# vitasoftAI/ImageRetrievalResearch

Measured on AMD Instinct MI355X. Metric: images/sec embed + queries/sec top-k@100k-gallery, EffNet-B3a 224^2, higher is better.
Workload: dtype bf16

## Files before the change

### imageretrievalresearch_amd/csrc/conv_kernels.hip

```cpp
#include "ops.h"

#include <stdlib.h>
#include <type_traits>

namespace mi355 {

typedef float f32x4 __attribute__((ext_vector_type(4)));
typedef unsigned u32x4 __attribute__((ext_vector_type(4)));
typedef unsigned u32x2 __attribute__((ext_vector_type(2)));

__device__ __forceinline__ void unpack8(u32x4 v, float* f) {
    f[0] = __uint_as_float(v.x << 16); f[1] = __uint_as_float(v.x & 0xffff0000u);
    f[2] = __uint_as_float(v.y << 16); f[3] = __uint_as_float(v.y & 0xffff0000u);
    f[4] = __uint_as_float(v.z << 16); f[5] = __uint_as_float(v.z & 0xffff0000u);
    f[6] = __uint_as_float(v.w << 16); f[7] = __uint_as_float(v.w & 0xffff0000u);
}
__device__ __forceinline__ u32x4 pack8(const float* f) {
    u32x4 o;
    o.x = pack2bf(f[0], f[1]); o.y = pack2bf(f[2], f[3]); o.z = pack2bf(f[4], f[5]); o.w = pack2bf(f[6], f[7]);
    return o;
}

__global__ __launch_bounds__(256) void k_stem(const float* __restrict__ x, const float* __restrict__ w,
                                              const float* __restrict__ bias, bf16_t* __restrict__ out, int H, int W,
                                              int Ho, int Wo, int Cout, int act) {
    const int b = blockIdx.z;
    const int ox = blockIdx.x * 32 + (threadIdx.x & 31);
    const int oy = blockIdx.y * 8 + (threadIdx.x >> 5);
    if (ox >= Wo || oy >= Ho) return;
    float p[27];
    const float* xb = x + (size_t)b * 3 * H * W;
#pragma unroll
    for (int ky = 0; ky < 3; ++ky) {
        const int iy = oy * 2 - 1 + ky;
#pragma unroll
        for (int kx = 0; kx < 3; ++kx) {
            const int ix = ox * 2 - 1 + kx;
            const bool ok = (iy >= 0 && iy < H && ix >= 0 && ix < W);
#pragma unroll
            for (int ci = 0; ci < 3; ++ci)
                p[(ky * 3 + kx) * 3 + ci] = ok ? xb[((size_t)ci * H + iy) * W + ix] : 0.f;
        }
    }
    bf16_t* o = out + (((size_t)b * Ho + oy) * Wo + ox) * Cout;
    for (int c0 = 0; c0 < Cout; c0 += 8) {
        float acc[8];
#pragma unroll
        for (int j = 0; j < 8; ++j) acc[j] = bias[c0 + j];
#pragma unroll
        for (int t = 0; t < 27; ++t) {
            const f32x4 w0 = *reinterpret_cast<const f32x4*>(&w[t * Cout + c0]);
            const f32x4 w1 = *reinterpret_cast<const f32x4*>(&w[t * Cout + c0 + 4]);
            acc[0] += p[t] * w0.x; acc[1] += p[t] * w0.y; acc[2] += p[t] * w0.z; acc[3] += p[t] * w0.w;
            acc[4] += p[t] * w1.x; acc[5] += p[t] * w1.y; acc[6] += p[t] * w1.z; acc[7] += p[t] * w1.w;
        }
        MI355_ACT_DISPATCH(act, {
_Pragma("unroll")
            for (int j = 0; j < 8; ++j) acc[j] = act_c<ACT>(acc[j]);
        })
        *reinterpret_cast<u32x4*>(o + c0) = pack8(acc);
    }
}

int launch_stem(const float* x, const float* w, const float* bias, bf16_t* out, int B, int H, int W, int Cout, int act,
                hipStream_t st) {
    MI355_REQUIRE(Cout % 8 == 0 && Cout <= 256, "stem: Cout=%d must be a multiple of 8 and <= 256", Cout);
    const int Ho = (H + 2 - 3) / 2 + 1, Wo = (W + 2 - 3) / 2 + 1;
    dim3 grid(cdiv(Wo, 32), cdiv(Ho, 8), B);
    hipLaunchKernelGGL(k_stem, grid, dim3(256), 0, st, x, w, bias, out, H, W, Ho, Wo, Cout, act);
    MI355_LAUNCH_CHECK();
    return OK;
}

struct StemU8Args {
    const unsigned char* img;
    int h, w, S, hp, vp, fill;
    float mean[3], stdv[3];
    const float* cw;
};
struct StemU8RaggedArgs : StemU8Args {
    const int64_t* desc;
    int b0;
};

template <bool CONV_INPUT, bool RAGGED>
__global__ __launch_bounds__(256) void k_stem_u8(const std::conditional_t<RAGGED, StemU8RaggedArgs, StemU8Args> a,
                                                 const float* __restrict__ w,
                                                 const float* __restrict__ bias, bf16_t* __restrict__ out, int Ho, int Wo,
                                                 int Cout, int act) {
    constexpr int PW = 67, PH = 19, CWD = 65, CHT = 17;
    __shared__ float scw[81];
    __shared__ float Pt[CONV_INPUT ? PH * PW * 3 : 1];
    __shared__ float Ct[CONV_INPUT ? CHT * CWD * 3 : 1];
    const int b = blockIdx.z;
    const int lx = threadIdx.x & 31, ly = threadIdx.x >> 5;
    const int ox = blockIdx.x * 32 + lx;
    const int oy = blockIdx.y * 8 + ly;
    StemU8Args g = a;
    if constexpr (RAGGED) {
        const int64_t* d = a.desc + (size_t)(a.b0 + b) * 3;
        g.img = a.img + d[0]; g.h = (int)d[1]; g.w = (int)d[2];
        g.hp = (a.S - g.w) / 2; g.vp = (a.S - g.h) / 2;
    }
    const unsigned char* ib = RAGGED ? g.img : g.img + (size_t)b * g.h * g.w * 3;
    auto pre = [&](int y, int x, int c) -> float {
        if (y < 0 || y >= g.S || x < 0 || x >= g.S) return 0.f;
        const int iy = y - g.vp, ix = x - g.hp;
        int v = g.fill;
        if (iy >= 0 && iy < g.h && ix >= 0 && ix < g.w) v = ib[((size_t)iy * g.w + ix) * 3 + c];
        return __fdiv_rn(__fsub_rn(__fdiv_rn((float)v, 255.0f), g.mean[c]), g.stdv[c]);
    };
    float p[27];
    if (!CONV_INPUT) {
        if (ox >= Wo || oy >= Ho) return;
#pragma unroll
        for (int ky = 0; ky < 3; ++ky)
#pragma unroll
            for (int kx = 0; kx < 3; ++kx)
#pragma unroll
                for (int ci = 0; ci < 3; ++ci) p[(ky * 3 + kx) * 3 + ci] = pre(oy * 2 - 1 + ky, ox * 2 - 1 + kx, ci);
    } else {
        if (threadIdx.x < 81) scw[threadIdx.x] = g.cw[threadIdx.x];
        const int y0 = blockIdx.y * 16 - 2, x0 = blockIdx.x * 64 - 2;
        for (int i = threadIdx.x; i < PH * PW; i += 256) {
            const int r = i / PW, c = i - r * PW;
#pragma unroll
            for (int ci = 0; ci < 3; ++ci) Pt[i * 3 + ci] = pre(y0 + r, x0 + c, ci);
        }
        __syncthreads();
        for (int i = threadIdx.x; i < CHT * CWD; i += 256) {
            const int r = i / CWD, c = i - r * CWD;
            const int y = y0 + 1 + r, x = x0 + 1 + c;
            float acc[3] = {0.f, 0.f, 0.f};
#pragma unroll
            for (int ci = 0; ci < 3; ++ci)
#pragma unroll
                for (int ky2 = 0; ky2 < 3; ++ky2)
#pragma unroll
                    for (int kx2 = 0; kx2 < 3; ++kx2) {
                        const float v = Pt[((r + ky2) * PW + c + kx2) * 3 + ci];
#pragma unroll
                        for (int co = 0; co < 3; ++co) acc[co] += v * scw[((co * 3 + ci) * 3 + ky2) * 3 + kx2];
                    }
            const bool in = y >= 0 && y < g.S && x >= 0 && x < g.S;
#pragma unroll
            for (int co = 0; co < 3; ++co) Ct[i * 3 + co] = in ? silu_f(acc[co]) : 0.f;
        }
        __syncthreads();
        if (ox >= Wo || oy >= Ho) return;
#pragma unroll
        for (int ky = 0; ky < 3; ++ky)
#pragma unroll
            for (int kx = 0; kx < 3; ++kx)
#pragma unroll
                for (int co = 0; co < 3; ++co) p[(ky * 3 + kx) * 3 + co] = Ct[((ly * 2 + ky) * CWD + lx * 2 + kx) * 3 + co];
    }
    bf16_t* o = out + (((size_t)b * Ho + oy) * Wo + ox) * Cout;
    for (int c0 = 0; c0 < Cout; c0 += 8) {
        float acc[8];
#pragma unroll
        for (int j = 0; j < 8; ++j) acc[j] = bias[c0 + j];
#pragma unroll
        for (int t = 0; t < 27; ++t) {
            const f32x4 w0 = *reinterpret_cast<const f32x4*>(&w[t * Cout + c0]);
            const f32x4 w1 = *reinterpret_cast<const f32x4*>(&w[t * Cout + c0 + 4]);
            acc[0] += p[t] * w0.x; acc[1] += p[t] * w0.y; acc[2] += p[t] * w0.z; acc[3] += p[t] * w0.w;
            acc[4] += p[t] * w1.x; acc[5] += p[t] * w1.y; acc[6] += p[t] * w1.z; acc[7] += p[t] * w1.w;
        }
        MI355_ACT_DISPATCH(act, {
_Pragma("unroll")
            for (int j = 0; j < 8; ++j) acc[j] = act_c<ACT>(acc[j]);
        })
        *reinterpret_cast<u32x4*>(o + c0) = pack8(acc);
    }
}

int launch_stem_u8(const unsigned char* img, int h, int w, int fill, const float* mean, const float* stdv,
                   const float* conv_w, const float* sw, const float* bias, bf16_t* out, int B, int Cout, int act,
                   hipStream_t st, const int64_t* desc, int b0) {
    MI355_REQUIRE(Cout % 8 == 0 && Cout <= 256, "stem: Cout=%d must be a multiple of 8 and <= 256", Cout);
    StemU8RaggedArgs r{};
    StemU8Args& a = r;
    a.img = img; a.h = h; a.w = w; a.S = h > w ? h : w; a.hp = (a.S - w) / 2; a.vp = (a.S - h) / 2; a.fill = fill;
    for (int c = 0; c < 3; ++c) { a.mean[c] = mean[c]; a.stdv[c] = stdv[c]; }
    a.cw = conv_w;
    r.desc = desc; r.b0 = b0;
    const int Ho = (a.S + 2 - 3) / 2 + 1, Wo = Ho;
    dim3 grid(cdiv(Wo, 32), cdiv(Ho, 8), B);
    if (desc) {
        if (conv_w) hipLaunchKernelGGL((k_stem_u8<true, true>), grid, dim3(256), 0, st, r, sw, bias, out, Ho, Wo, Cout, act);
        else hipLaunchKernelGGL((k_stem_u8<false, true>), grid, dim3(256), 0, st, r, sw, bias, out, Ho, Wo, Cout, act);
    } else if (conv_w) {
        hipLaunchKernelGGL((k_stem_u8<true, false>), grid, dim3(256), 0, st, a, sw, bias, out, Ho, Wo, Cout, act);
    } else {
        hipLaunchKernelGGL((k_stem_u8<false, false>), grid, dim3(256), 0, st, a, sw, bias, out, Ho, Wo, Cout, act);
    }
    MI355_LAUNCH_CHECK();
    return OK;
}

#ifndef MI355_DW_PX
#define MI355_DW_PX 4
#endif
constexpr int DW_PX = MI355_DW_PX;

int dw_pool_blocks(int Ho, int Wo, int C) {
    const long items = (long)(C / 8) * cdiv(Wo, DW_PX) * Ho;
    return cdiv(items, 256);
}

template <int KS, int S>
__global__ __launch_bounds__(256) void k_dwconv(const bf16_t* __restrict__ in, const bf16_t* __restrict__ w,
                                                const float* __restrict__ bias, bf16_t* __restrict__ out,
                                                float* __restrict__ pool_partial, int B, int nblk, int H, int W, int C,
                                                int Ho, int Wo, int act) {
    constexpr int PAD = KS / 2;
    constexpr int IW = (DW_PX - 1) * S + KS;
    __shared__ float red[256][8];
    const int CG = C >> 3;
    const int strips = (Wo + DW_PX - 1) / DW_PX;
    const int xcd = blockIdx.x & 7;
    const int seq = blockIdx.x >> 3;
    const int b = xcd + 8 * (seq / nblk);
    const int blk = seq - (seq / nblk) * nblk;
    if (b >= B) return;
    const long item = (long)blk * 256 + threadIdx.x;
    const long nitems = (long)CG * strips * Ho;
    const bool live = item < nitems;
    const int cg = (int)(item % CG);
    const long rest = item / CG;
    const int sx = (int)(rest % strips);
    const int oy = (int)(rest / strips);
    const int ox0 = sx * DW_PX;
    const int c0 = cg * 8;

    float acc[DW_PX][8];
    float psum[8];
#pragma unroll
    for (int j = 0; j < 8; ++j) psum[j] = 0.f;

    if (live) {
        float bs[8];
        {
            const f32x4 b0 = *reinterpret_cast<const f32x4*>(bias + c0);
            const f32x4 b1 = *reinterpret_cast<const f32x4*>(bias + c0 + 4);
            bs[0] = b0.x; bs[1] = b0.y; bs[2] = b0.z; bs[3] = b0.w; bs[4] = b1.x; bs[5] = b1.y; bs[6] = b1.z; bs[7] = b1.w;
        }
#pragma unroll
        for (int p = 0; p < DW_PX; ++p)
#pragma unroll
            for (int j = 0; j < 8; ++j) acc[p][j] = bs[j];

        const bf16_t* inb = in + (size_t)b * H * W * C + c0;
#pragma unroll
        for (int ky = 0; ky < KS; ++ky) {
            const int iy = oy * S - PAD + ky;
            if (iy < 0 || iy >= H) continue;
            float wk[KS][8];
#pragma unroll
            for (int kx = 0; kx < KS; ++kx)
                unpack8(*reinterpret_cast<const u32x4*>(w + (size_t)(ky * KS + kx) * C + c0), wk[kx]);
            const bf16_t* row = inb + (size_t)iy * W * C;
#pragma unroll
            for (int i = 0; i < IW; ++i) {
                const int ix = ox0 * S - PAD + i;
                if (ix < 0 || ix >= W) continue;
                float v[8];
                unpack8(*reinterpret_cast<const u32x4*>(row + (size_t)ix * C), v);
#pragma unroll
                for (int p = 0; p < DW_PX; ++p) {
                    const int kx = i - p * S;
                    if (kx >= 0 && kx < KS) {
#pragma unroll
                        for (int j = 0; j < 8; ++j) acc[p][j] += wk[kx][j] * v[j];
                    }
                }
            }
        }
        bf16_t* o = out + (((size_t)b * Ho + oy) * Wo + ox0) * C + c0;
        MI355_ACT_DISPATCH(act, {
_Pragma("unroll")
            for (int p = 0; p < DW_PX; ++p)
_Pragma("unroll")
                for (int j = 0; j < 8; ++j) acc[p][j] = act_c<ACT>(acc[p][j]);
        })
#pragma unroll
        for (int p = 0; p < DW_PX; ++p) {
            if (ox0 + p < Wo) {
#pragma unroll
                for (int j = 0; j < 8; ++j) psum[j] += acc[p][j];
                if (C >= 64) __builtin_nontemporal_store(pack8(acc[p]), reinterpret_cast<u32x4*>(o + (size_t)p * C));
                else *reinterpret_cast<u32x4*>(o + (size_t)p * C) = pack8(acc[p]);
            }
        }
    }

    if (pool_partial != nullptr) {
#pragma unroll
        for (int j = 0; j < 8; ++j) red[threadIdx.x][j] = psum[j];
        __syncthreads();
        const int ncg = CG < 256 ? CG : 256;
        if ((int)threadIdx.x < ncg) {
            float s[8];
#pragma unroll
            for (int j = 0; j < 8; ++j) s[j] = 0.f;
            for (int u = threadIdx.x; u < 256; u += CG) {
#pragma unroll
                for (int j = 0; j < 8; ++j) s[j] += red[u][j];
            }
            const int my_cg = (int)(((long)blk * 256 + threadIdx.x) % CG);
            float* pp = pool_partial + ((size_t)b * nblk + blk) * C + my_cg * 8;
            *reinterpret_cast<f32x4*>(pp) = (f32x4){s[0], s[1], s[2], s[3]};
            *reinterpret_cast<f32x4*>(pp + 4) = (f32x4){s[4], s[5], s[6], s[7]};
        }
        if (CG > 256) {
            const int first = (int)(((long)blk * 256) % CG);
            for (int t = 256 + threadIdx.x; t < CG; t += 256) {
                const int z = (first + t) % CG;
                float* pp = pool_partial + ((size_t)b * nblk + blk) * C + z * 8;
                *reinterpret_cast<f32x4*>(pp) = (f32x4){0.f, 0.f, 0.f, 0.f};
                *reinterpret_cast<f32x4*>(pp + 4) = (f32x4){0.f, 0.f, 0.f, 0.f};
            }
        }
    }
}

template <int KS, int PX>
__global__ __launch_bounds__(256) void k_dw_tiled(const bf16_t* __restrict__ in, const bf16_t* __restrict__ w,
                                                  const float* __restrict__ bias, bf16_t* __restrict__ out,
                                                  float* __restrict__ pool_partial, int H, int W, int C, int TH, int CGC,
                                                  int nbands, int act) {
    constexpr int PAD = KS / 2;
    constexpr int IW = PX - 1 + KS;
    extern __shared__ __attribute__((aligned(16))) bf16_t tile[];
    const int b = blockIdx.y;
    const int band = blockIdx.x % nbands, chunk = blockIdx.x / nbands;
    const int oy0 = band * TH;
    const int th = min(TH, H - oy0);
    const int IH = TH + KS - 1, EW = W + 2 * PAD + (PX - 1);
    const int cg0 = chunk * CGC;
    const int CG = C >> 3;
    const int ncg = min(CGC, CG - cg0);
    const int PS = CGC * 8;
    const bf16_t* inb = in + (size_t)b * H * W * C;
    for (int id = threadIdx.x; id < IH * EW * CGC; id += 256) {
        const int cg = id % CGC;
        const int px = id / CGC;
        const int r = px / EW, x = px - r * EW;
        const int iy = oy0 - PAD + r, ix = x - PAD;
        u32x4 v = {0u, 0u, 0u, 0u};
        if (cg < ncg && iy >= 0 && iy < H && ix >= 0 && ix < W)
            v = *reinterpret_cast<const u32x4*>(inb + ((size_t)iy * W + ix) * C + (cg0 + cg) * 8);
        *reinterpret_cast<u32x4*>(&tile[(size_t)px * PS + cg * 8]) = v;
    }
    __syncthreads();

    const int strips = (W + PX - 1) / PX;
    const int nitems = CGC * strips * th;
    float psum[8];
#pragma unroll
    for (int j = 0; j < 8; ++j) psum[j] = 0.f;
    for (int item = threadIdx.x; item < nitems; item += 256) {
        const int cg = item % CGC;
        const int rest = item / CGC;
        const int sx = rest % strips, oyl = rest / strips;
        if (cg >= ncg) continue;
        const int ox0 = sx * PX;
        const int c0 = (cg0 + cg) * 8;
        float acc[PX][8];
        {
            const f32x4 b0 = *reinterpret_cast<const f32x4*>(bias + c0);
            const f32x4 b1 = *reinterpret_cast<const f32x4*>(bias + c0 + 4);
// ... 585 lines not shown
```

### imageretrievalresearch_amd/csrc/gemm_bf16.hip

```cpp
#include "ops.h"
#include "../../include/mi355_retrieval.h"

#include <stdlib.h>

namespace mi355 {

typedef __bf16 bf16x8 __attribute__((ext_vector_type(8)));
typedef float f32x4 __attribute__((ext_vector_type(4)));
typedef unsigned u32x4 __attribute__((ext_vector_type(4)));
typedef unsigned u32x2 __attribute__((ext_vector_type(2)));

__device__ __forceinline__ float lo_bf(unsigned u) { return __uint_as_float(u << 16); }
__device__ __forceinline__ float hi_bf(unsigned u) { return __uint_as_float(u & 0xffff0000u); }

__device__ __forceinline__ u32x4 gate_chunk(u32x4 v, const float* __restrict__ gp, int relu6) {
    const f32x4 g0 = *reinterpret_cast<const f32x4*>(gp);
    const f32x4 g1 = *reinterpret_cast<const f32x4*>(gp + 4);
    float f[8] = {lo_bf(v.x) * g0.x, hi_bf(v.x) * g0.y, lo_bf(v.y) * g0.z, hi_bf(v.y) * g0.w,
                  lo_bf(v.z) * g1.x, hi_bf(v.z) * g1.y, lo_bf(v.w) * g1.z, hi_bf(v.w) * g1.w};
    if (relu6) {
#pragma unroll
        for (int i = 0; i < 8; ++i) f[i] = fminf(fmaxf(f[i], 0.f), 6.f);
    }
    u32x4 o;
// ... 647 lines not shown
        if (row < Npad && c * 8 < g.ldw) v = *reinterpret_cast<const u32x4*>(g.W + (size_t)row * g.ldw + c * 8);
        *reinterpret_cast<u32x4*>(&Wsh[row * WLD + c * 8]) = v;
    }
    for (int n = tid; n < NT * 16; n += 512) sbias[n] = n < Npad ? g.bias[n] : 0.f;
    for (int id = lane; id < 16 * (ALD / 8); id += 64) *reinterpret_cast<u32x4*>(&As[id * 8]) = (u32x4){0u, 0u, 0u, 0u};
    __syncthreads();

    const int fr = lane & 15, fq = lane >> 4;
    const int kc = g.K >> 3;
    const int nchunk = 16 * kc;
    const int ntiles = (g.M + 15) >> 4;
    const int stride = gridDim.x * NW;
    int img = -1;
    u32x4 sv[KST];
    auto stage_load = [&](int tile) {
#pragma unroll
        for (int i = 0; i < KST; ++i) {
            const int id = min(lane + 64 * i, nchunk - 1);
            const int row = id / kc, c = id - row * kc;
            const int m = min(tile * 16 + row, g.M - 1);
            sv[i] = *reinterpret_cast<const u32x4*>(g.A + (size_t)m * g.lda + c * 8);
        }
        __builtin_amdgcn_sched_barrier(0);
    };
    int tile = blockIdx.x * NW + wave;
    if (tile < ntiles) stage_load(tile);
    for (; tile < ntiles; tile += stride) {
        if (g.gate) {
            const int im = (tile * 16) / g.rows_per_img;
            if (im != img) {
                img = im;
                for (int k4 = lane; k4 * 4 < g.K; k4 += 64)
                    *reinterpret_cast<f32x4*>(&Gs[k4 * 4]) = *reinterpret_cast<const f32x4*>(g.gate + (size_t)im * g.gate_ld + k4 * 4);
            }
        }
#pragma unroll
        for (int i = 0; i < KST; ++i) {
            const int id = lane + 64 * i;
            if (id < nchunk) {
                const int row = id / kc, c = id - row * kc;
                u32x4 v = sv[i];
                if (g.gate) v = gate_chunk(v, Gs + c * 8, g.a_relu6);
                else if (g.a_relu6) v = relu6_chunk(v);
                *reinterpret_cast<u32x4*>(&As[row * ALD + c * 8]) = v;
            }
        }
        if (tile + stride < ntiles) stage_load(tile + stride);
        f32x4 acc[NT];
#pragma unroll
        for (int ni = 0; ni < NT; ++ni) acc[ni] = (f32x4){0.f, 0.f, 0.f, 0.f};
#pragma unroll
        for (int ks = 0; ks < KST; ++ks) {
            const bf16x8 af = *reinterpret_cast<const bf16x8*>(&As[fr * ALD + ks * 32 + fq * 8]);
#pragma unroll
            for (int ni = 0; ni < NT; ++ni) {
                const bf16x8 wf = *reinterpret_cast<const bf16x8*>(&Wsh[(ni * 16 + fr) * WLD + ks * 32 + fq * 8]);
                acc[ni] = __builtin_amdgcn_mfma_f32_16x16x32_bf16(wf, af, acc[ni], 0, 0, 0);
            }
        }
        MI355_ACT_DISPATCH(g.act, {
_Pragma("unroll")
            for (int ni = 0; ni < NT; ++ni) {
                const f32x4 bb = *reinterpret_cast<const f32x4*>(&sbias[ni * 16 + fq * 4]);
                acc[ni].x = act_c<ACT>(acc[ni].x + bb.x); acc[ni].y = act_c<ACT>(acc[ni].y + bb.y);
                acc[ni].z = act_c<ACT>(acc[ni].z + bb.z); acc[ni].w = act_c<ACT>(acc[ni].w + bb.w);
            }
        })
        const int m = tile * 16 + fr;
#pragma unroll
        for (int ni = 0; ni < NT; ++ni) {
            const int n = ni * 16 + fq * 4;
            float v[4] = {acc[ni].x, acc[ni].y, acc[ni].z, acc[ni].w};
            if (g.res && m < g.M && n < g.N) {
                if (n + 3 < g.res_n) {
                    const u32x2 rr = *reinterpret_cast<const u32x2*>(g.res + (size_t)m * g.ldr + n);
                    v[0] += lo_bf(rr.x); v[1] += hi_bf(rr.x); v[2] += lo_bf(rr.y); v[3] += hi_bf(rr.y);
                } else {
#pragma unroll
                    for (int r = 0; r < 4; ++r)
                        if (n + r < g.res_n) v[r] += bf2f(g.res[(size_t)m * g.ldr + n + r]);
                }
            }
            u32x2 o;
            o.x = pack2bf(v[0], v[1]);
            o.y = pack2bf(v[2], v[3]);
            *reinterpret_cast<u32x2*>(&Cs[fr * CLD + n]) = o;
        }
        constexpr int CPR = NT * 2;
#pragma unroll
        for (int i = 0; i < (16 * CPR + 63) / 64; ++i) {
            const int id = lane + 64 * i;
            const int row = id / CPR, c = id - row * CPR;
            const int mm = tile * 16 + row;
            if (id < 16 * CPR && mm < g.M && c * 8 < g.N)
                *reinterpret_cast<u32x4*>((bf16_t*)g.out + (size_t)mm * g.ldo + c * 8) =
                    *reinterpret_cast<const u32x4*>(&Cs[row * CLD + c * 8]);
        }
    }
}

template <int NT, int KST>
static int launch_proj_cfg(const GemmArgs& a, hipStream_t st) {
    constexpr int KP = KST * 32;
    const size_t lds = (size_t)NT * 16 * (KP + 8) * 2 + (size_t)NT * 16 * 4 +
                       (size_t)8 * (16 * (KP + 8) * 2 + 16 * (NT * 16 + 8) * 2 + KP * 4);
    static bool attr_done[MI355_MAX_DEVICES] = {false};
    if (first_time_on_this_device(attr_done)) {
        MI355_CHECK_HIP(hipFuncSetAttribute((const void*)k_proj_lds<NT, KST>, hipFuncAttributeMaxDynamicSharedMemorySize,
                                            160 * 1024));
    }
    const int ntiles = cdiv(a.M, 16);
    int blocks = cdiv(ntiles, 8);
    if (blocks > 256 * 6) blocks = 256 * 6;
    hipLaunchKernelGGL((k_proj_lds<NT, KST>), dim3(blocks), dim3(512), lds, st, a);
    MI355_LAUNCH_CHECK();
    return OK;
}

static int try_launch_proj(const GemmArgs& a, hipStream_t st, int* nt_out) {
    if (a.out_f32 || a.M < (1 << 19) || a.N % 8 || a.ldo % 8 || a.N > 64 || a.K > 288 || a.lda != a.K) return -1;
    if (a.gate && (a.rows_per_img % 16 != 0 || a.gate_ld % 4 != 0)) return -1;
    const int kst = (a.K + 31) / 32, nt = (a.N + 15) / 16;
#define PROJ_CASE(NTV, KSTV) if (nt == NTV && kst == KSTV) { *nt_out = NTV; return launch_proj_cfg<NTV, KSTV>(a, st); }
    PROJ_CASE(2, 1); PROJ_CASE(2, 2); PROJ_CASE(2, 5); PROJ_CASE(2, 6); PROJ_CASE(3, 6); PROJ_CASE(3, 9); PROJ_CASE(2, 9);
    PROJ_CASE(4, 8); PROJ_CASE(3, 5);
#undef PROJ_CASE
    return -1;
}

static int try_launch_stream(const GemmArgs& a, hipStream_t st, int* nt_out) {
    if (a.out_f32 || a.M < 4096 || a.N % 8 || a.ldo % 8 || a.gate || a.a_relu6) return -1;
    const int kst = (a.K + 31) / 32;
    const int nt = (a.N + 15) / 16;
    *nt_out = nt;
    if (kst == 1 && nt == 9) return launch_stream_cfg<9, 1>(a, st);
    if (kst == 1 && nt == 12) return launch_stream_cfg<12, 1>(a, st);
    return -1;
}

constexpr int SK_KC = 256, SK_BM = 64, SK_BN = 64, SK_LD = SK_KC + 8;
constexpr size_t SK_MAX_BYTES = (size_t)64 << 20;

int gemm_splitk_chunks(long M, int rows_per_img, int N, int K) {
    if (M > 16384 || rows_per_img > 196 || K < 512 || N < 64 || N % 8 || gemm_splitk_bytes(M, N, K) > SK_MAX_BYTES) return 0;
    return (K + SK_KC - 1) / SK_KC;
}
size_t gemm_splitk_bytes(long M, int N, int K) {
    return (size_t)((K + SK_KC - 1) / SK_KC) * (size_t)M * (size_t)((N + 15) & ~15) * sizeof(float);
}

__global__ __launch_bounds__(256) void k_gemm_splitk(const GemmArgs g, float* __restrict__ ws) {
    extern __shared__ __attribute__((aligned(16))) bf16_t sksm[];
    bf16_t* As = sksm;
    bf16_t* Ws = sksm + SK_BM * SK_LD;
    const int tid = threadIdx.x, lane = tid & 63, wave = tid >> 6;
    const int n0 = blockIdx.x * SK_BN, m0 = blockIdx.y * SK_BM, k0 = blockIdx.z * SK_KC;
    const int Npad = (g.N + 15) & ~15;
    u32x4 ra[8], rw[8];
#pragma unroll
    for (int i = 0; i < 8; ++i) {
        const int id = tid + 256 * i;
        const int row = id >> 5, c = id & 31;
        const int k = k0 + c * 8;
        const int m = min(m0 + row, g.M - 1), kk = min(k, g.K - 8);
        ra[i] = *reinterpret_cast<const u32x4*>(g.A + (size_t)m * g.lda + kk);
        const int n = min(n0 + row, Npad - 1), kw = min(k, g.ldw - 8);
        rw[i] = *reinterpret_cast<const u32x4*>(g.W + (size_t)n * g.ldw + kw);
    }
#pragma unroll
    for (int i = 0; i < 8; ++i) {
        const int id = tid + 256 * i;
        const int row = id >> 5, c = id & 31;
        const int k = k0 + c * 8;
        u32x4 v = ra[i];
        if (m0 + row < g.M && k < g.K) {
            if (g.gate) v = gate_chunk(v, g.gate + (size_t)((m0 + row) / g.rows_per_img) * g.gate_ld + k, g.a_relu6);
            else if (g.a_relu6) v = relu6_chunk(v);
        } else {
            v = (u32x4){0u, 0u, 0u, 0u};
        }
        *reinterpret_cast<u32x4*>(&As[row * SK_LD + c * 8]) = v;
        u32x4 w = rw[i];
        if (n0 + row >= Npad || k >= g.ldw) w = (u32x4){0u, 0u, 0u, 0u};
        *reinterpret_cast<u32x4*>(&Ws[row * SK_LD + c * 8]) = w;
    }
    __syncthreads();
    const int fr = lane & 15, fq = lane >> 4;
    const int wm = wave >> 1, wn = wave & 1;
    f32x4 acc[2][2];
#pragma unroll
    for (int j = 0; j < 2; ++j)
#pragma unroll
        for (int i = 0; i < 2; ++i) acc[j][i] = (f32x4){0.f, 0.f, 0.f, 0.f};
#pragma unroll
    for (int ks = 0; ks < SK_KC / 32; ++ks) {
        bf16x8 af[2], wf[2];
#pragma unroll
        for (int i = 0; i < 2; ++i) af[i] = *reinterpret_cast<const bf16x8*>(&As[(wm * 32 + i * 16 + fr) * SK_LD + ks * 32 + fq * 8]);
#pragma unroll
        for (int j = 0; j < 2; ++j) wf[j] = *reinterpret_cast<const bf16x8*>(&Ws[(wn * 32 + j * 16 + fr) * SK_LD + ks * 32 + fq * 8]);
#pragma unroll
        for (int j = 0; j < 2; ++j)
#pragma unroll
            for (int i = 0; i < 2; ++i) acc[j][i] = __builtin_amdgcn_mfma_f32_16x16x32_bf16(wf[j], af[i], acc[j][i], 0, 0, 0);
    }
    float* wsk = ws + (size_t)blockIdx.z * g.M * Npad;
#pragma unroll
    for (int i = 0; i < 2; ++i) {
        const int m = m0 + wm * 32 + i * 16 + fr;
#pragma unroll
        for (int j = 0; j < 2; ++j) {
            const int n = n0 + wn * 32 + j * 16 + fq * 4;
            if (m < g.M && n < Npad) *reinterpret_cast<f32x4*>(wsk + (size_t)m * Npad + n) = acc[j][i];
        }
    }
}

__global__ __launch_bounds__(256) void k_splitk_reduce(const GemmArgs g, const float* __restrict__ ws, int nchunks) {
    const int Npad = (g.N + 15) & ~15, n4s = Npad >> 2;
    const long t = (long)blockIdx.x * 256 + threadIdx.x;
    if (t >= (long)g.M * n4s) return;
    const int m = (int)(t / n4s), n = (int)(t - (long)m * n4s) * 4;
    if (n >= g.N) return;
    f32x4 s = *reinterpret_cast<const f32x4*>(ws + (size_t)m * Npad + n);
    for (int c = 1; c < nchunks; ++c) {
        const f32x4 p = *reinterpret_cast<const f32x4*>(ws + ((size_t)c * g.M + m) * Npad + n);
        s.x += p.x; s.y += p.y; s.z += p.z; s.w += p.w;
    }
    const f32x4 bb = *reinterpret_cast<const f32x4*>(g.bias + n);
    float v[4] = {apply_act(s.x + bb.x, g.act), apply_act(s.y + bb.y, g.act), apply_act(s.z + bb.z, g.act), apply_act(s.w + bb.w, g.act)};
    if (g.res) {
#pragma unroll
        for (int r = 0; r < 4; ++r)
            if (n + r < g.res_n) v[r] += bf2f(g.res[(size_t)m * g.ldr + n + r]);
    }
    u32x2 o;
    o.x = pack2bf(v[0], v[1]);
    o.y = pack2bf(v[2], v[3]);
    *reinterpret_cast<u32x2*>((bf16_t*)g.out + (size_t)m * g.ldo + n) = o;
}

static int launch_splitk(const GemmArgs& a, int nchunks, hipStream_t st) {
    const size_t lds = (size_t)(SK_BM + SK_BN) * SK_LD * 2;
    static bool attr_done[MI355_MAX_DEVICES] = {false};
    if (first_time_on_this_device(attr_done)) {
        MI355_CHECK_HIP(hipFuncSetAttribute((const void*)k_gemm_splitk, hipFuncAttributeMaxDynamicSharedMemorySize, (int)lds));
    }
    const int Npad = (a.N + 15) & ~15;
    hipLaunchKernelGGL(k_gemm_splitk, dim3((unsigned)cdiv(Npad, SK_BN), (unsigned)cdiv(a.M, SK_BM), (unsigned)nchunks), dim3(256), lds, st,
                       a, a.splitk_ws);
    MI355_LAUNCH_CHECK();
    hipLaunchKernelGGL(k_splitk_reduce, dim3((unsigned)cdiv((long)a.M * (Npad / 4), 256)), dim3(256), 0, st, a,
                       (const float*)a.splitk_ws, nchunks);
    MI355_LAUNCH_CHECK();
    return OK;
}

static int pick_nt(int N, int max_nt = 12) {
    static const int opts[] = {2, 3, 4, 6, 8, 9, 12};
    int best = 2;
    double best_cost = 1e30;
    for (int nt : opts) {
        if (nt > max_nt) continue;
        const int bn = nt * 16;
        const int tiles = (N + bn - 1) / bn;
        const double cost = (double)tiles * bn * (1.0 + 24.0 / bn) + 8.0 * tiles;
        if (cost < best_cost) { best_cost = cost; best = nt; }
    }
    return best;
}

template <int WM, int NT, int BK>
static int launch_cfg(const GemmArgs& a, hipStream_t st) {
    constexpr int BM = 64 * WM, BN = NT * 16, LD = BK + 8;
    constexpr size_t stage = (size_t)2 * (BM + BN) * LD * 2, ctile = (size_t)BM * (BN + 8) * 2;
    constexpr size_t lds = stage > ctile ? stage : ctile;
    static bool attr_done[MI355_MAX_DEVICES] = {false};
    if (first_time_on_this_device(attr_done)) {
        MI355_CHECK_HIP(hipFuncSetAttribute((const void*)k_gemm_bf16<WM, NT, BK>,
                                            hipFuncAttributeMaxDynamicSharedMemorySize, (int)lds));
    }
    const int n_tiles = cdiv(a.N, BN);
    const int m_tiles = cdiv(a.M, BM);
    const long nwg = (long)n_tiles * m_tiles;
    MI355_REQUIRE(nwg < (1l << 31), "gemm: grid too large");
    hipLaunchKernelGGL((k_gemm_bf16<WM, NT, BK>), dim3((unsigned)nwg), dim3(256), lds, st, a, n_tiles, (int)nwg);
    MI355_LAUNCH_CHECK();
    return OK;
}

template <int WM, int BK>
static int launch_nt(const GemmArgs& a, int nt, hipStream_t st) {
    switch (nt) {
        case 2: return launch_cfg<WM, 2, BK>(a, st);
        case 3: return launch_cfg<WM, 3, BK>(a, st);
        case 4: return launch_cfg<WM, 4, BK>(a, st);
        case 6: return launch_cfg<WM, 6, BK>(a, st);
        case 8: return launch_cfg<WM, 8, BK>(a, st);
        case 9: return launch_cfg<WM, 9, BK>(a, st);
        default: return launch_cfg<WM, 12, BK>(a, st);
    }
}

template <int ACT>
__global__ __launch_bounds__(256) void k_head_gap(const bf16_t* __restrict__ A, int lda, const bf16_t* __restrict__ W, int ldw,
                                                  const float* __restrict__ bias, float* __restrict__ pooled,
                                                  bf16_t* __restrict__ pooled_bf16, int ldp, int HW, int N, int K) {
    constexpr int TLD = 132;
    __shared__ __attribute__((aligned(16))) float T[64 * TLD];
    const int tid = threadIdx.x, lane = tid & 63, wave = tid >> 6;
    const int fr = lane & 15, fq = lane >> 4;
    const int wm = wave >> 1, wn = wave & 1;
    const int b = blockIdx.y, n0 = blockIdx.x * 128;
    const int Npad = (N + 15) & ~15;
    const bf16_t* Ab = A + (size_t)b * HW * lda;
    const bf16_t* arow[2];
    const bf16_t* wrow[4];
#pragma unroll
    for (int mi = 0; mi < 2; ++mi) arow[mi] = Ab + (size_t)min(wm * 32 + mi * 16 + fr, HW - 1) * lda;
#pragma unroll
    for (int ni = 0; ni < 4; ++ni) wrow[ni] = W + (size_t)min(n0 + wn * 64 + ni * 16 + fr, Npad - 1) * ldw;
    f32x4 acc[4][2];
#pragma unroll
    for (int ni = 0; ni < 4; ++ni)
#pragma unroll
        for (int mi = 0; mi < 2; ++mi) acc[ni][mi] = (f32x4){0.f, 0.f, 0.f, 0.f};
    const int nks = (K + 31) >> 5;
    u32x4 af[2][2], wf[2][4];
    auto load = [&](int s, int ks) {
        const int ka = min(ks * 32 + fq * 8, lda - 8), kw = ks * 32 + fq * 8;
#pragma unroll
        for (int mi = 0; mi < 2; ++mi) af[s][mi] = *reinterpret_cast<const u32x4*>(arow[mi] + ka);
#pragma unroll
        for (int ni = 0; ni < 4; ++ni) wf[s][ni] = *reinterpret_cast<const u32x4*>(wrow[ni] + kw);
    };
    load(0, 0);
    for (int ks = 0; ks < nks; ks += 2) {
        if (ks + 1 < nks) load(1, ks + 1);
#pragma unroll
        for (int ni = 0; ni < 4; ++ni)
#pragma unroll
            for (int mi = 0; mi < 2; ++mi)
                acc[ni][mi] = __builtin_amdgcn_mfma_f32_16x16x32_bf16(*reinterpret_cast<bf16x8*>(&wf[0][ni]), *reinterpret_cast<bf16x8*>(&af[0][mi]), acc[ni][mi], 0, 0, 0);
        if (ks + 1 < nks) {
            if (ks + 2 < nks) load(0, ks + 2);
#pragma unroll
            for (int ni = 0; ni < 4; ++ni)
#pragma unroll
                for (int mi = 0; mi < 2; ++mi)
                    acc[ni][mi] = __builtin_amdgcn_mfma_f32_16x16x32_bf16(*reinterpret_cast<bf16x8*>(&wf[1][ni]), *reinterpret_cast<bf16x8*>(&af[1][mi]), acc[ni][mi], 0, 0, 0);
        }
    }
#pragma unroll
    for (int ni = 0; ni < 4; ++ni) {
        const int nl = wn * 64 + ni * 16 + fq * 4;
        f32x4 bb = {0.f, 0.f, 0.f, 0.f};
        if (n0 + nl < Npad) bb = *reinterpret_cast<const f32x4*>(bias + n0 + nl);
#pragma unroll
        for (int mi = 0; mi < 2; ++mi) {
            const int ml = wm * 32 + mi * 16 + fr;
            f32x4 v;
            v.x = bf2f(f2bf(act_c<ACT>(acc[ni][mi].x + bb.x))); v.y = bf2f(f2bf(act_c<ACT>(acc[ni][mi].y + bb.y)));
            v.z = bf2f(f2bf(act_c<ACT>(acc[ni][mi].z + bb.z))); v.w = bf2f(f2bf(act_c<ACT>(acc[ni][mi].w + bb.w)));
            *reinterpret_cast<f32x4*>(&T[ml * TLD + nl]) = v;
        }
    }
    __syncthreads();
    if (tid < 128 && n0 + tid < N) {
        float s = 0.f;
        for (int i = 0; i < HW; ++i) s += T[i * TLD + tid];
        s *= 1.0f / (float)HW;
        pooled[(size_t)b * ldp + n0 + tid] = s;
        if (pooled_bf16) pooled_bf16[(size_t)b * ldp + n0 + tid] = f2bf(s);
    }
}

bool head_gap_supported(int HW, int N, int K, int lda, int ldw, int act) {
    return HW >= 1 && HW <= 64 && K >= 32 && K <= 512 && lda % 8 == 0 && lda >= 8 && ldw % 32 == 0 && ldw >= ((K + 31) & ~31) && N % 8 == 0 &&
           (act == ACT_SILU || act == ACT_NONE);
}

int launch_head_gap(const bf16_t* A, int lda, const bf16_t* W, int ldw, const float* bias, float* pooled, bf16_t* pooled_bf16,
                    int ldp, int B, int HW, int N, int K, int act, hipStream_t st) {
    MI355_REQUIRE(head_gap_supported(HW, N, K, lda, ldw, act), "head_gap: unsupported shape HW=%d N=%d K=%d", HW, N, K);
    const dim3 grid((unsigned)cdiv(N, 128), (unsigned)B);
    if (act == ACT_SILU) hipLaunchKernelGGL(k_head_gap<ACT_SILU>, grid, dim3(256), 0, st, A, lda, W, ldw, bias, pooled, pooled_bf16, ldp, HW, N, K);
    else hipLaunchKernelGGL(k_head_gap<ACT_NONE>, grid, dim3(256), 0, st, A, lda, W, ldw, bias, pooled, pooled_bf16, ldp, HW, N, K);
    MI355_LAUNCH_CHECK();
    return OK;
}

int launch_gemm_bf16(const GemmArgs& a, hipStream_t st, int* path) {
    auto ran = [&](int p, int e) { if (path && e == OK) *path = p; return e; };
    if (path) *path = 0;
    MI355_REQUIRE(a.M >= 1 && a.N >= 1 && a.K >= 1, "gemm: bad shape M=%d N=%d K=%d", a.M, a.N, a.K);
    MI355_REQUIRE(a.K % 8 == 0 && a.lda % 8 == 0 && a.ldw % 32 == 0, "gemm: K=%d lda=%d ldw=%d alignment", a.K, a.lda,
                  a.ldw);
    MI355_REQUIRE(a.out_f32 || (a.ldo % 8 == 0 && a.N % 8 == 0), "gemm: bf16 output needs N, ldo multiples of 8 (N=%d ldo=%d)",
                  a.N, a.ldo);
    MI355_REQUIRE(!a.res || a.ldr % 4 == 0, "gemm: residual stride %d must be a multiple of 4", a.ldr);
    static const int use_splitk = getenv("MI355_GEMM_SPLITK") ? atoi(getenv("MI355_GEMM_SPLITK")) : 1;
    if (use_splitk && a.splitk_ws && !a.out_f32 && a.ldo % 4 == 0 && !a.ln_stats) {
        const int nch = gemm_splitk_chunks(a.M_sel > 0 ? a.M_sel : a.M, a.rows_per_img > 0 ? a.rows_per_img : a.M, a.N, a.K);
        if (nch >= 2 && gemm_splitk_bytes(a.M, a.N, a.K) <= a.splitk_ws_bytes && (!a.gate || a.gate_ld % 4 == 0))
            return ran(MI355_GEMM_PATH_SPLITK, launch_splitk(a, nch, st));
    }
    const int use_wide = getenv("MI355_GEMM_WIDE") ? atoi(getenv("MI355_GEMM_WIDE")) : 0;
    if (use_wide && gemm_wide_supported(a)) return ran(MI355_GEMM_PATH_WIDE, launch_gemm_wide(a, st));
    if (a.ln_stats) {
        const bool ktail_ = (a.K % 64 != 0) || (a.ldw % 64 != 0);
        MI355_REQUIRE(a.zeros && a.K >= 128 && a.N >= 96 && a.M >= 1024 && ((uintptr_t)a.A % 16 == 0) && a.lda % 8 == 0 && !a.gate &&
                      !a.a_relu6 && !ktail_, "gemm: LayerNorm folding needs the DMA-tiled kernel (M=%d N=%d K=%d)", a.M, a.N, a.K);
    }
    static const int short_min_k = getenv("MI355_GEMM_SHORT_MIN_K") ? atoi(getenv("MI355_GEMM_SHORT_MIN_K")) : 64;
    if (a.zeros && a.K >= short_min_k && a.K < 128 && a.N >= 2 * a.K && a.N >= 96 && a.M >= 32768 && ((uintptr_t)a.A % 16 == 0) &&
        a.lda % 8 == 0 && !a.gate && !a.a_relu6 && !a.ln_stats) {
        const bool ktail32 = (a.K % 32 != 0) || (a.ldw % 32 != 0);
        return ktail32 ? ran(MI355_GEMM_PATH_BIG32_KTAIL, launch_big<false, true, 32>(a, st))
                       : ran(MI355_GEMM_PATH_BIG32, launch_big<false, false, 32>(a, st));
    }
    if (a.zeros && a.K >= 128 && a.N >= 64 && a.M >= 1024 && ((uintptr_t)a.A % 16 == 0) && a.lda % 8 == 0 &&
        (!a.gate || a.gate_ld >= a.K)) {
        const bool fits = a.N <= BG_BN ? a.N >= 72 : (long)a.N * 16 >= (long)cdiv(a.N, BG_BN) * BG_BN * 10;
        const bool ktail = (a.K % 64 != 0) || (a.ldw % 64 != 0);
        if ((a.gate || a.a_relu6) && fits)
            return ktail ? ran(MI355_GEMM_PATH_BIG_GATED_KTAIL, launch_big<true, true>(a, st))
                         : ran(MI355_GEMM_PATH_BIG_GATED, launch_big<true, false>(a, st));
        if (!a.gate && !a.a_relu6 && a.N >= 96) {
            static const int short_k = getenv("MI355_GEMM_SHORT_K") ? atoi(getenv("MI355_GEMM_SHORT_K")) : 128;
            if (!ktail && a.K <= short_k && a.N >= a.K && a.M >= 32768) return ran(MI355_GEMM_PATH_BIG32, launch_big<false, false, 32>(a, st));
            return ktail ? ran(MI355_GEMM_PATH_BIG_KTAIL, launch_big<false, true>(a, st)) : ran(MI355_GEMM_PATH_BIG, launch_big<false, false>(a, st));
        }
    }
    static const int use_stream = getenv("MI355_GEMM_STREAM") ? atoi(getenv("MI355_GEMM_STREAM")) : 1;
    if (use_stream) {
        int nt = 0;
        const int e = try_launch_stream(a, st, &nt);
        if (e >= 0) return ran(MI355_GEMM_PATH_STREAM | nt << 8, e);
    }
    static const int use_proj = getenv("MI355_GEMM_PROJ") ? atoi(getenv("MI355_GEMM_PROJ")) : 1;
    if (use_proj) {
        int nt = 0;
        const int e = try_launch_proj(a, st, &nt);
        if (e >= 0) return ran(MI355_GEMM_PATH_PROJ | nt << 8, e);
    }
    const int small_cap = a.N % 64 == 0 ? 4 : 9;
    const int nt = pick_nt(a.N, a.K <= 64 ? small_cap : 12);
    if (a.M <= 64)
        return a.K >= 64 ? ran(MI355_GEMM_PATH_TILE_M64_BK64 | nt << 8, launch_nt<1, 64>(a, nt, st))
                         : ran(MI355_GEMM_PATH_TILE_M64_BK32 | nt << 8, launch_nt<1, 32>(a, nt, st));
    return ran(MI355_GEMM_PATH_TILE | nt << 8, launch_nt<2, 32>(a, nt, st));
}

}
```

Measured before the change: 59770.

## Tile stem conv input through LDS and stage head-GAP weights in shared memory

```diff
diff --git a/imageretrievalresearch_amd/csrc/conv_kernels.hip b/imageretrievalresearch_amd/csrc/conv_kernels.hip
--- a/imageretrievalresearch_amd/csrc/conv_kernels.hip
+++ b/imageretrievalresearch_amd/csrc/conv_kernels.hip
@@ -21,28 +21,57 @@
     return o;
 }
 
+constexpr int STEM_TW = 16, STEM_TH = 16;
+constexpr int STEM_IR = 2 * STEM_TH + 1, STEM_IC = 2 * STEM_TW + 4;
+
+static size_t stem_lds_bytes(int Cout) {
+    return (size_t)3 * STEM_IR * STEM_IC * sizeof(float) + (size_t)4 * 64 * Cout * sizeof(bf16_t);
+}
+
 __global__ __launch_bounds__(256) void k_stem(const float* __restrict__ x, const float* __restrict__ w,
                                               const float* __restrict__ bias, bf16_t* __restrict__ out, int H, int W,
                                               int Ho, int Wo, int Cout, int act) {
+    extern __shared__ __attribute__((aligned(16))) float stem_sm[];
+    float* xin = stem_sm;
+    const int tid = threadIdx.x, lane = tid & 63, wave = tid >> 6;
+    bf16_t* strip = reinterpret_cast<bf16_t*>(stem_sm + 3 * STEM_IR * STEM_IC) + (size_t)wave * 64 * Cout;
     const int b = blockIdx.z;
-    const int ox = blockIdx.x * 32 + (threadIdx.x & 31);
-    const int oy = blockIdx.y * 8 + (threadIdx.x >> 5);
-    if (ox >= Wo || oy >= Ho) return;
+    const int ox0 = blockIdx.x * STEM_TW, oy0 = blockIdx.y * STEM_TH;
+    const int ix0 = 2 * ox0 - 4, iy0 = 2 * oy0 - 1;
+    const float* xb = x + (size_t)b * 3 * H * W;
+    if ((W & 3) == 0) {
+        constexpr int G = STEM_IC / 4, NV = (3 * STEM_IR * G + 255) / 256;
+        f32x4 v[NV];
+#pragma unroll
+        for (int j = 0; j < NV; ++j) {
+            const int i = tid + 256 * j;
+            const int row = i / G, g = i - row * G;
+            const int ci = row / STEM_IR, iy = iy0 + row - ci * STEM_IR, ix = ix0 + g * 4;
+            v[j] = (f32x4){0.f, 0.f, 0.f, 0.f};
+            if (i < 3 * STEM_IR * G && iy >= 0 && iy < H && ix >= 0 && ix < W)
+                v[j] = *reinterpret_cast<const f32x4*>(xb + ((size_t)ci * H + iy) * W + ix);
+        }
+#pragma unroll
+        for (int j = 0; j < NV; ++j)
+            if (tid + 256 * j < 3 * STEM_IR * G) *reinterpret_cast<f32x4*>(&xin[(tid + 256 * j) * 4]) = v[j];
+    } else {
+        for (int i = tid; i < 3 * STEM_IR * STEM_IC; i += 256) {
+            const int row = i / STEM_IC, c = i - row * STEM_IC;
+            const int ci = row / STEM_IR, iy = iy0 + row - ci * STEM_IR, ix = ix0 + c;
+            xin[i] = (iy >= 0 && iy < H && ix >= 0 && ix < W) ? xb[((size_t)ci * H + iy) * W + ix] : 0.f;
+        }
+    }
+    __syncthreads();
+    const int lx = tid & (STEM_TW - 1), ly = tid / STEM_TW;
     float p[27];
-    const float* xb = x + (size_t)b * 3 * H * W;
-#pragma unroll
-    for (int ky = 0; ky < 3; ++ky) {
-        const int iy = oy * 2 - 1 + ky;
-#pragma unroll
-        for (int kx = 0; kx < 3; ++kx) {
-            const int ix = ox * 2 - 1 + kx;
-            const bool ok = (iy >= 0 && iy < H && ix >= 0 && ix < W);
+#pragma unroll
+    for (int ky = 0; ky < 3; ++ky)
+#pragma unroll
+        for (int kx = 0; kx < 3; ++kx)
 #pragma unroll
             for (int ci = 0; ci < 3; ++ci)
-                p[(ky * 3 + kx) * 3 + ci] = ok ? xb[((size_t)ci * H + iy) * W + ix] : 0.f;
-        }
-    }
-    bf16_t* o = out + (((size_t)b * Ho + oy) * Wo + ox) * Cout;
+                p[(ky * 3 + kx) * 3 + ci] = xin[(ci * STEM_IR + 2 * ly + ky) * STEM_IC + 2 * lx + 3 + kx];
+    bf16_t* o = strip + (size_t)lane * Cout;
     for (int c0 = 0; c0 < Cout; c0 += 8) {
         float acc[8];
 #pragma unroll
@@ -60,14 +89,29 @@
         })
         *reinterpret_cast<u32x4*>(o + c0) = pack8(acc);
     }
+    const int cpp = Cout / 8;
+    const int cpr = STEM_TW * cpp;
+    const int nx = min(STEM_TW, Wo - ox0);
+    for (int id = lane; id < 4 * cpr; id += 64) {
+        const int r = id / cpr, c = id - r * cpr;
+        const int oy = oy0 + wave * 4 + r;
+        if (oy < Ho && c < nx * cpp)
+            *reinterpret_cast<u32x4*>(out + (((size_t)b * Ho + oy) * Wo + ox0) * Cout + (size_t)c * 8) =
+                *reinterpret_cast<const u32x4*>(strip + (size_t)id * 8);
+    }
 }
 
 int launch_stem(const float* x, const float* w, const float* bias, bf16_t* out, int B, int H, int W, int Cout, int act,
                 hipStream_t st) {
     MI355_REQUIRE(Cout % 8 == 0 && Cout <= 256, "stem: Cout=%d must be a multiple of 8 and <= 256", Cout);
     const int Ho = (H + 2 - 3) / 2 + 1, Wo = (W + 2 - 3) / 2 + 1;
-    dim3 grid(cdiv(Wo, 32), cdiv(Ho, 8), B);
-    hipLaunchKernelGGL(k_stem, grid, dim3(256), 0, st, x, w, bias, out, H, W, Ho, Wo, Cout, act);
+    const size_t lds = stem_lds_bytes(Cout);
+    static bool attr_done[MI355_MAX_DEVICES] = {};
+    if (lds > 65536 && first_time_on_this_device(attr_done))
+        MI355_CHECK_HIP(hipFuncSetAttribute((const void*)k_stem, hipFuncAttributeMaxDynamicSharedMemorySize,
+                                            (int)stem_lds_bytes(256)));
+    dim3 grid(cdiv(Wo, STEM_TW), cdiv(Ho, STEM_TH), B);
+    hipLaunchKernelGGL(k_stem, grid, dim3(256), lds, st, x, w, bias, out, H, W, Ho, Wo, Cout, act);
     MI355_LAUNCH_CHECK();
     return OK;
 }
diff --git a/imageretrievalresearch_amd/csrc/gemm_bf16.hip b/imageretrievalresearch_amd/csrc/gemm_bf16.hip
--- a/imageretrievalresearch_amd/csrc/gemm_bf16.hip
+++ b/imageretrievalresearch_amd/csrc/gemm_bf16.hip
@@ -973,76 +973,104 @@
     }
 }
 
-template <int ACT>
+constexpr int HG_NT = 128;
+constexpr int HG_SLD = HG_NT + 8;
+
+static int head_gap_wld(int K) { return ((K + 31) & ~31) + 8; }
+static size_t head_gap_lds_bytes(int K) {
+    return (size_t)HG_NT * head_gap_wld(K) * sizeof(bf16_t) + (size_t)4 * 16 * HG_SLD * sizeof(bf16_t);
+}
+
+template <int ACT, int KSMAX>
 __global__ __launch_bounds__(256) void k_head_gap(const bf16_t* __restrict__ A, int lda, const bf16_t* __restrict__ W, int ldw,
                                                   const float* __restrict__ bias, float* __restrict__ pooled,
-                                                  bf16_t* __restrict__ pooled_bf16, int ldp, int HW, int N, int K) {
-    constexpr int TLD = 132;
-    __shared__ __attribute__((aligned(16))) float T[64 * TLD];
+                                                  bf16_t* __restrict__ pooled_bf16, int ldp, int B, int HW, int N, int K) {
+    extern __shared__ __attribute__((aligned(16))) bf16_t hg_sm[];
     const int tid = threadIdx.x, lane = tid & 63, wave = tid >> 6;
     const int fr = lane & 15, fq = lane >> 4;
-    const int wm = wave >> 1, wn = wave & 1;
-    const int b = blockIdx.y, n0 = blockIdx.x * 128;
+    const int n0 = blockIdx.x * HG_NT;
     const int Npad = (N + 15) & ~15;
+    const int nks = (K + 31) >> 5;
+    const int WLD = nks * 32 + 8;
+    bf16_t* Ws = hg_sm;
+    bf16_t* strip = hg_sm + HG_NT * WLD + wave * 16 * HG_SLD;
+    {
+        const int cpr = nks * 4;
+        for (int i = tid; i < HG_NT * cpr; i += 256) {
+            const int r = i / cpr, c = i - r * cpr;
+            *reinterpret_cast<u32x4*>(&Ws[r * WLD + c * 8]) =
+                *reinterpret_cast<const u32x4*>(W + (size_t)min(n0 + r, Npad - 1) * ldw + c * 8);
+        }
+    }
+    __syncthreads();
+    const int b = blockIdx.y * 4 + wave;
+    if (b >= B) return;
     const bf16_t* Ab = A + (size_t)b * HW * lda;
-    const bf16_t* arow[2];
-    const bf16_t* wrow[4];
-#pragma unroll
-    for (int mi = 0; mi < 2; ++mi) arow[mi] = Ab + (size_t)min(wm * 32 + mi * 16 + fr, HW - 1) * lda;
-#pragma unroll
-    for (int ni = 0; ni < 4; ++ni) wrow[ni] = W + (size_t)min(n0 + wn * 64 + ni * 16 + fr, Npad - 1) * ldw;
-    f32x4 acc[4][2];
-#pragma unroll
-    for (int ni = 0; ni < 4; ++ni)
-#pragma unroll
-        for (int mi = 0; mi < 2; ++mi) acc[ni][mi] = (f32x4){0.f, 0.f, 0.f, 0.f};
-    const int nks = (K + 31) >> 5;
-    u32x4 af[2][2], wf[2][4];
+    const bf16_t* arow[4];
+#pragma unroll
+    for (int mi = 0; mi < 4; ++mi) arow[mi] = Ab + (size_t)min(mi * 16 + fr, HW - 1) * lda;
+    f32x4 acc[8][4];
+#pragma unroll
+    for (int ni = 0; ni < 8; ++ni)
+#pragma unroll
+        for (int mi = 0; mi < 4; ++mi) acc[ni][mi] = (f32x4){0.f, 0.f, 0.f, 0.f};
+    u32x4 af[3][4];
     auto load = [&](int s, int ks) {
-        const int ka = min(ks * 32 + fq * 8, lda - 8), kw = ks * 32 + fq * 8;
-#pragma unroll
-        for (int mi = 0; mi < 2; ++mi) af[s][mi] = *reinterpret_cast<const u32x4*>(arow[mi] + ka);
-#pragma unroll
-        for (int ni = 0; ni < 4; ++ni) wf[s][ni] = *reinterpret_cast<const u32x4*>(wrow[ni] + kw);
+        const int ka = min(ks * 32 + fq * 8, lda - 8);
+#pragma unroll
+        for (int mi = 0; mi < 4; ++mi) af[s][mi] = *reinterpret_cast<const u32x4*>(arow[mi] + ka);
     };
     load(0, 0);
-    for (int ks = 0; ks < nks; ks += 2) {
-        if (ks + 1 < nks) load(1, ks + 1);
-#pragma unroll
-        for (int ni = 0; ni < 4; ++ni)
-#pragma unroll
-            for (int mi = 0; mi < 2; ++mi)
-                acc[ni][mi] = __builtin_amdgcn_mfma_f32_16x16x32_bf16(*reinterpret_cast<bf16x8*>(&wf[0][ni]), *reinterpret_cast<bf16x8*>(&af[0][mi]), acc[ni][mi], 0, 0, 0);
-        if (ks + 1 < nks) {
-            if (ks + 2 < nks) load(0, ks + 2);
-#pragma unroll
-            for (int ni = 0; ni < 4; ++ni)
-#pragma unroll
-                for (int mi = 0; mi < 2; ++mi)
-                    acc[ni][mi] = __builtin_amdgcn_mfma_f32_16x16x32_bf16(*reinterpret_cast<bf16x8*>(&wf[1][ni]), *reinterpret_cast<bf16x8*>(&af[1][mi]), acc[ni][mi], 0, 0, 0);
-        }
-    }
-#pragma unroll
-    for (int ni = 0; ni < 4; ++ni) {
-        const int nl = wn * 64 + ni * 16 + fq * 4;
-        f32x4 bb = {0.f, 0.f, 0.f, 0.f};
-        if (n0 + nl < Npad) bb = *reinterpret_cast<const f32x4*>(bias + n0 + nl);
-#pragma unroll
-        for (int mi = 0; mi < 2; ++mi) {
-            const int ml = wm * 32 + mi * 16 + fr;
-            f32x4 v;
-            v.x = bf2f(f2bf(act_c<ACT>(acc[ni][mi].x + bb.x))); v.y = bf2f(f2bf(act_c<ACT>(acc[ni][mi].y + bb.y)));
-            v.z = bf2f(f2bf(act_c<ACT>(acc[ni][mi].z + bb.z))); v.w = bf2f(f2bf(act_c<ACT>(acc[ni][mi].w + bb.w)));
-            *reinterpret_cast<f32x4*>(&T[ml * TLD + nl]) = v;
-        }
-    }
-    __syncthreads();
-    if (tid < 128 && n0 + tid < N) {
-        float s = 0.f;
-        for (int i = 0; i < HW; ++i) s += T[i * TLD + tid];
-        s *= 1.0f / (float)HW;
-        pooled[(size_t)b * ldp + n0 + tid] = s;
-        if (pooled_bf16) pooled_bf16[(size_t)b * ldp + n0 + tid] = f2bf(s);
+    if (nks > 1) load(1, 1);
+#pragma unroll
+    for (int ks = 0; ks < KSMAX; ++ks) {
+        if (ks < nks) {
+            if (ks + 2 < nks) load((ks + 2) % 3, ks + 2);
+#pragma unroll
+            for (int ni = 0; ni < 8; ++ni) {
+                const u32x4 wf = *reinterpret_cast<const u32x4*>(&Ws[(ni * 16 + fr) * WLD + ks * 32 + fq * 8]);
+#pragma unroll
+                for (int mi = 0; mi < 4; ++mi)
+                    acc[ni][mi] = __builtin_amdgcn_mfma_f32_16x16x32_bf16(*reinterpret_cast<const bf16x8*>(&wf),
+                                                                          *reinterpret_cast<const bf16x8*>(&af[ks % 3][mi]),
+                                                                          acc[ni][mi], 0, 0, 0);
+            }
+        }
+    }
+    f32x4 bb[8];
+#pragma unroll
+    for (int ni = 0; ni < 8; ++ni) {
+        const int n = n0 + ni * 16 + fq * 4;
+        bb[ni] = n < Npad ? *reinterpret_cast<const f32x4*>(bias + n) : (f32x4){0.f, 0.f, 0.f, 0.f};
+    }
+    float s0 = 0.f, s1 = 0.f;
+#pragma unroll
+    for (int mi = 0; mi < 4; ++mi) {
+        if (mi * 16 >= HW) break;
+#pragma unroll
+        for (int ni = 0; ni < 8; ++ni) {
+            const f32x4 a = acc[ni][mi];
+            u32x2 o;
+            o.x = pack2bf(act_c<ACT>(a.x + bb[ni].x), act_c<ACT>(a.y + bb[ni].y));
+            o.y = pack2bf(act_c<ACT>(a.z + bb[ni].z), act_c<ACT>(a.w + bb[ni].w));
+            *reinterpret_cast<u32x2*>(&strip[fr * HG_SLD + ni * 16 + fq * 4]) = o;
+        }
+        const int np = min(16, HW - mi * 16);
+        for (int i = 0; i < np; ++i) {
+            const unsigned v = *reinterpret_cast<const unsigned*>(&strip[i * HG_SLD + 2 * lane]);
+            s0 += __uint_as_float(v << 16);
+            s1 += __uint_as_float(v & 0xffff0000u);
+        }
+    }
+    const int n = n0 + 2 * lane;
+    if (n < N) {
+        s0 *= 1.0f / (float)HW;
+        s1 *= 1.0f / (float)HW;
+        *reinterpret_cast<float2*>(&pooled[(size_t)b * ldp + n]) = make_float2(s0, s1);
+        if (pooled_bf16) {
+            pooled_bf16[(size_t)b * ldp + n] = f2bf(s0);
+            pooled_bf16[(size_t)b * ldp + n + 1] = f2bf(s1);
+        }
     }
 }
 
@@ -1051,14 +1079,29 @@
            (act == ACT_SILU || act == ACT_NONE);
 }
 
+template <int ACT, int KSMAX>
+static int launch_head_gap_cfg(const bf16_t* A, int lda, const bf16_t* W, int ldw, const float* bias, float* pooled,
+                               bf16_t* pooled_bf16, int ldp, int B, int HW, int N, int K, hipStream_t st) {
+    static bool attr_done[MI355_MAX_DEVICES] = {};
+    if (first_time_on_this_device(attr_done))
+        MI355_CHECK_HIP(hipFuncSetAttribute((const void*)k_head_gap<ACT, KSMAX>, hipFuncAttributeMaxDynamicSharedMemorySize,
+                                            (int)head_gap_lds_bytes(KSMAX * 32)));
+    const dim3 grid((unsigned)cdiv(N, HG_NT), (unsigned)cdiv(B, 4));
+    hipLaunchKernelGGL((k_head_gap<ACT, KSMAX>), grid, dim3(256), head_gap_lds_bytes(K), st, A, lda, W, ldw, bias, pooled,
+                       pooled_bf16, ldp, B, HW, N, K);
+    MI355_LAUNCH_CHECK();
+    return OK;
+}
+
 int launch_head_gap(const bf16_t* A, int lda, const bf16_t* W, int ldw, const float* bias, float* pooled, bf16_t* pooled_bf16,
                     int ldp, int B, int HW, int N, int K, int act, hipStream_t st) {
     MI355_REQUIRE(head_gap_supported(HW, N, K, lda, ldw, act), "head_gap: unsupported shape HW=%d N=%d K=%d", HW, N, K);
-    const dim3 grid((unsigned)cdiv(N, 128), (unsigned)B);
-    if (act == ACT_SILU) hipLaunchKernelGGL(k_head_gap<ACT_SILU>, grid, dim3(256), 0, st, A, lda, W, ldw, bias, pooled, pooled_bf16, ldp, HW, N, K);
-    else hipLaunchKernelGGL(k_head_gap<ACT_NONE>, grid, dim3(256), 0, st, A, lda, W, ldw, bias, pooled, pooled_bf16, ldp, HW, N, K);
-    MI355_LAUNCH_CHECK();
-    return OK;
+    const bool small_k = K <= 12 * 32;
+    if (act == ACT_SILU)
+        return small_k ? launch_head_gap_cfg<ACT_SILU, 12>(A, lda, W, ldw, bias, pooled, pooled_bf16, ldp, B, HW, N, K, st)
+                       : launch_head_gap_cfg<ACT_SILU, 16>(A, lda, W, ldw, bias, pooled, pooled_bf16, ldp, B, HW, N, K, st);
+    return small_k ? launch_head_gap_cfg<ACT_NONE, 12>(A, lda, W, ldw, bias, pooled, pooled_bf16, ldp, B, HW, N, K, st)
+                   : launch_head_gap_cfg<ACT_NONE, 16>(A, lda, W, ldw, bias, pooled, pooled_bf16, ldp, B, HW, N, K, st);
 }
 
 int launch_gemm_bf16(const GemmArgs& a, hipStream_t st, int* path) {
```

After: 60970, median of 6. +2.0%, better.
